# scverse/squidpy

Measured on AMD Instinct MI355X. Metric: nhood_enrichment permutations/sec (1e6 spots x 30 clusters), higher is better.
Workload: dtype u8 labels / u32 counts / i64 moments; 1 GPU; nhood_enrichment: 1000000 spots (1000x1000 hex grid, nnz=5992002), 30 clusters, 10000 permutations per step per GPU, on-device Philox-keyed label shuffles; collective=none

## Files before the change

### squidpy_amd/csrc/sqgr_nhood.hip

```cpp
#include "sqgr_common.h"
#include "sqgr_rng.h"
#include "sqgr_shuffle.h"
#include "sqgr_pcg.h"

#include <algorithm>
#include <cstdlib>
#include <type_traits>

namespace sqgr {

constexpr int COUNT_THREADS = 1024;
constexpr size_t LDS_BUDGET = 160 * 1024;

__host__ __device__ constexpr int key_words_per_row(int B, int n_libs) {
    return n_libs * ((B / FEISTEL_GROUP) * 8 + (B / 2) * 2) < (B / 2) * 8 ? (B / 2) * 8 : n_libs * ((B / FEISTEL_GROUP) * 8 + (B / 2) * 2);
}

__global__ void k_keygen(uint64_t seed, int64_t perm0, int nrows, int B, int n_libs, uint32_t* __restrict__ keys) {
    const int items = B / FEISTEL_GROUP + B / 2;
    const int64_t t = blockIdx.x * (int64_t)blockDim.x + threadIdx.x;
    if (t >= (int64_t)nrows * n_libs * items) return;
    const int item = (int)(t % items);
    const uint32_t lib = (uint32_t)((t / items) % n_libs);
    const int64_t row = t / ((int64_t)items * n_libs);
// ... 55 lines not shown
    if (pw == 16) {
        *reinterpret_cast<uint4*>(batch_base + (size_t)i * 16) = make_uint4(w0, w1, w2, w3);
    } else if (pw == 8) {
        *reinterpret_cast<uint2*>(batch_base + (size_t)i * 8) = make_uint2(w0, w1);
        *reinterpret_cast<uint2*>(batch_base + (size_t)n * 8 + (size_t)i * 8) = make_uint2(w2, w3);
    } else if (pw == 4) {
        uint32_t* d = reinterpret_cast<uint32_t*>(batch_base) + i;
        d[0] = w0; d[(size_t)n] = w1; d[(size_t)2 * n] = w2; d[(size_t)3 * n] = w3;
    } else if (pw == 2) {
        uint16_t* d = reinterpret_cast<uint16_t*>(batch_base) + i;
        const uint32_t w[4] = {w0, w1, w2, w3};
#pragma unroll
        for (int q = 0; q < 8; ++q) d[(size_t)q * n] = (uint16_t)(w[q >> 1] >> (16 * (q & 1)));
    } else {
        uint8_t* d = batch_base + i;
        const uint32_t w[4] = {w0, w1, w2, w3};
#pragma unroll
        for (int q = 0; q < 16; ++q) d[(size_t)q * n] = (uint8_t)(w[q >> 2] >> (8 * (q & 3)));
    }
}

template <int B, bool HAS_LIBS, bool SMALLK>
__global__ __launch_bounds__(256) void k_shuffle(int64_t n, const uint32_t* __restrict__ cum, int kpad, int blk_words, int K,
                                                 const uint32_t* __restrict__ keys, LibDom dom0, int n_libs, int nrows,
                                                 const int32_t* __restrict__ lib_of, const int32_t* __restrict__ rank_of,
                                                 const LibDom* __restrict__ libdoms, uint8_t* __restrict__ slab_all, int pw,
                                                 const int32_t* __restrict__ spot_of) {
    extern __shared__ uint32_t s_lds[];
    uint32_t* s_cum = s_lds + blk_words;
    for (int t = threadIdx.x; t < n_libs * kpad; t += 256) s_cum[t] = cum[t];
    for (int t = threadIdx.x; t < blk_words; t += 256) s_lds[t] = cum[n_libs * kpad + t];
    __syncthreads();
    constexpr int NG = B / FEISTEL_GROUP;
    const int row0 = (NG == 2) ? blockIdx.y : 2 * blockIdx.y;
    const int row1 = (NG == 2) ? row0 : min(row0 + 1, nrows - 1);
    const bool store1 = (NG == 2) || row0 + 1 < nrows;
    const size_t row_words = key_words_per_row(B, n_libs);
    const uint32_t* kgA = keys + (size_t)row0 * row_words;
    const uint32_t* kgB = (NG == 2) ? kgA + (size_t)n_libs * 8 : keys + (size_t)row1 * row_words;
    const uint32_t* ksA = keys + (size_t)row0 * row_words + (size_t)NG * n_libs * 8;
    const uint32_t* ksB = (NG == 2) ? ksA + (size_t)(FEISTEL_GROUP / 2) * n_libs * 2
                                    : keys + (size_t)row1 * row_words + (size_t)NG * n_libs * 8;
    const uint32_t zero = 0;
    const uint32_t sent_add = (uint32_t)(128 - K) * 0x01010101u;
    for (int64_t i = blockIdx.x * (int64_t)blockDim.x + threadIdx.x; i < n; i += (int64_t)gridDim.x * blockDim.x) {
    LibDom ld = dom0;
    uint32_t x0 = (uint32_t)i, lib = 0;
    if (HAS_LIBS) {
        lib = (uint32_t)lib_of[i];
        ld = libdoms[lib];
        x0 = (uint32_t)rank_of[i];
    } else if (spot_of) {
        x0 = (uint32_t)spot_of[i];
    }
    const FeistelDomain dom = ld.dom;
    const uint32_t* tab = s_cum + lib * kpad + 1;
    typedef __attribute__((address_space(3))) const uint32_t lds_word;
    const uint32_t blk_base = HAS_LIBS ? ld.aoff * 4u : 0u;
    auto blk_at = [&](uint32_t byte_off) { return *reinterpret_cast<lds_word*>((uintptr_t)(blk_base + byte_off)); };
    const uint32_t a0 = x0 / dom.B, b0 = x0 - a0 * dom.B;

    u16x2 ga = (u16x2)((unsigned short)a0), gb = (u16x2)((unsigned short)b0);
    {
        uint32_t kp[8];
#pragma unroll
        for (int r = 0; r < 8; ++r) kp[r] = (kgA[(size_t)lib * 8 + r] & 0xFFFFu) | (kgB[(size_t)lib * 8 + r] & 0xFFFF0000u);
        const uint32_t* const pg[1] = {kp};
        bool need0 = true, need1 = true;
        do {
            u16x2 na[1] = {ga}, nb[1] = {gb};
            feistel_rounds<1>(na, nb, dom, pg);
            if (need0) { ga.x = na[0].x; gb.x = nb[0].x; }
            if (need1) { ga.y = na[0].y; gb.y = nb[0].y; }
            need0 = __umul24((uint32_t)ga.x, dom.B) + (uint32_t)gb.x >= dom.n;
            need1 = __umul24((uint32_t)ga.y, dom.B) + (uint32_t)gb.y >= dom.n;
        } while (need0 | need1);
    }
    auto emit_group = [&](const u16x2 gsa, const u16x2 gsb, const uint32_t* ks, uint32_t (&out)[4]) {
#pragma unroll
        for (int w = 0; w < FEISTEL_GROUP / 4; ++w) {
            uint32_t word = 0;
            uint32_t apk[2], bpk[2];
#pragma unroll
            for (int jj = 0; jj < 2; ++jj) {
                const uint32_t* const pk[1] = {ks + ((size_t)(w * 2 + jj) * n_libs + lib) * 2};
                u16x2 a[1] = {gsa}, b[1] = {gsb};
                sigma_rounds<1>(a, b, dom, pk);
                apk[jj] = __builtin_bit_cast(uint32_t, a[0]);
                bpk[jj] = __builtin_bit_cast(uint32_t, b[0]);
                const uint32_t a4 = apk[jj] << 2;
                const uint32_t e0 = blk_at(a4 & 0xFFFFu);
                const uint32_t e1 = blk_at(a4 >> 16);
                if (jj == 0) {
                    put_label<0, 0>(word, e0, bpk[jj], zero);
                    put_label<1, 1>(word, e1, bpk[jj], zero);
                } else {
                    put_label<2, 0>(word, e0, bpk[jj], zero);
                    put_label<3, 1>(word, e1, bpk[jj], zero);
                }
            }
            bool sentinel;
            if constexpr (SMALLK) {
                sentinel = ((word + sent_add) & 0x80808080u) != 0;
            } else {
                const uint32_t k = (uint32_t)K;
                sentinel = k > 255u || (word & 0xFFu) >= k || ((word >> 8) & 0xFFu) >= k || ((word >> 16) & 0xFFu) >= k || (word >> 24) >= k;
            }
            if (sentinel) {
#pragma unroll
                for (int j = 0; j < 4; ++j) {
                    if (K <= 255 && ((word >> (8 * j)) & 0xFFu) < (uint32_t)K) continue;
                    const int jj = j >> 1, sh = (j & 1) * 16;
                    const uint32_t* sk = ks + ((size_t)(w * 2 + jj) * n_libs + lib) * 2;
                    const uint32_t k0 = (sk[0] >> sh) & 0xFFFFu, k1 = (sk[1] >> sh) & 0xFFFFu;
                    uint32_t a = (apk[jj] >> sh) & 0xFFFFu, b = (bpk[jj] >> sh) & 0xFFFFu;
                    uint32_t x = a * dom.B + b;
                    while (x >= dom.n) {
                        uint32_t t = b + feistel_F1(a, k0, dom.bsh);
                        t = t >= dom.B ? t - dom.B : t;
                        b = t >= dom.B ? t - dom.B : t;
                        a = (a + feistel_F1(b, k1, dom.ash)) & (dom.A - 1u);
                        x = a * dom.B + b;
                    }
                    const uint32_t e = blk_at(a * 4u);
                    uint32_t l = (e & 0xFFFFu) + (b >= (e >> 16) ? 1u : 0u);
                    if (l >= (uint32_t)K) {
                        l = K <= 255 ? (e >> 8) & 0xFFu : 0u;
                        while (x >= tab[l]) ++l;
                    }
                    word = (word & ~(0xFFu << (8 * j))) | (l << (8 * j));
                }
            }
            out[w] = word;
        }
    };
    uint32_t outA[4], outB[4];
    emit_group((u16x2)(ga.x), (u16x2)(gb.x), ksA, outA);
    if (store1) emit_group((u16x2)(ga.y), (u16x2)(gb.y), ksB, outB);
    if constexpr (NG == 2) {
        uint4* dst = reinterpret_cast<uint4*>(slab_all + ((size_t)row0 * n + i) * B);
        dst[0] = make_uint4(outA[0], outA[1], outA[2], outA[3]);
        dst[1] = make_uint4(outB[0], outB[1], outB[2], outB[3]);
    } else {
        slab_store16(slab_all + (size_t)row0 * n * 16, n, i, pw, outA[0], outA[1], outA[2], outA[3]);
        if (store1) slab_store16(slab_all + (size_t)row1 * n * 16, n, i, pw, outB[0], outB[1], outB[2], outB[3]);
    }
    }
}

constexpr int SHUF_TAB_THREADS = 1024;
constexpr uint32_t SHUF_TAB_MAX_A = 1024;
constexpr int SHUF_TAB_BLOCKS_PER_CU = 20;
constexpr int SHUF_TAB_MIN_TRIPS = 16;
template <bool SMALLK>
__global__ __launch_bounds__(SHUF_TAB_THREADS, 8) void k_shuffle_tab(int64_t n, const uint32_t* __restrict__ cum, int kpad, int blk_words, int K,
                                                                  const uint32_t* __restrict__ keys, LibDom dom0, int nrows,
                                                                  uint8_t* __restrict__ slab_all, int pw, const int32_t* __restrict__ spot_of,
                                                                  int tab_word0) {
    extern __shared__ uint32_t s_lds[];
    uint32_t* s_cum = s_lds + blk_words;
    for (int t = threadIdx.x; t < kpad; t += SHUF_TAB_THREADS) s_cum[t] = cum[t];
    for (int t = threadIdx.x; t < blk_words; t += SHUF_TAB_THREADS) s_lds[t] = cum[kpad + t];
    const FeistelDomain dom = dom0.dom;
    const int row0 = 2 * blockIdx.y;
    const int row1 = min(row0 + 1, nrows - 1);
    const bool store1 = row0 + 1 < nrows;
    constexpr size_t row_words = key_words_per_row(16, 1);
    const uint32_t* kgA = keys + (size_t)row0 * row_words;
    const uint32_t* kgB = keys + (size_t)row1 * row_words;
    const uint32_t* ksA = kgA + 8;
    const uint32_t* ksB = kgB + 8;
    const u16x2 BB = (u16x2)((unsigned short)dom.B);
    {
        const u16x2 bsh = (u16x2)((unsigned short)dom.bsh);
        const int words = (int)dom.A * 8;
        for (int idx = threadIdx.x; idx < words; idx += SHUF_TAB_THREADS) {
            const u16x2 av = (u16x2)((unsigned short)(idx >> 3));
            const int t = idx & 7;
            u16x2 fa = feistel_F2(av, __builtin_bit_cast(u16x2, ksA[t * 2]), bsh);
            u16x2 fb = feistel_F2(av, __builtin_bit_cast(u16x2, ksB[t * 2]), bsh);
            fa = __builtin_elementwise_min(fa, (u16x2)(fa - BB));
            fb = __builtin_elementwise_min(fb, (u16x2)(fb - BB));
            s_lds[tab_word0 + idx] = __builtin_bit_cast(uint32_t, fa);
            s_lds[tab_word0 + words + idx] = __builtin_bit_cast(uint32_t, fb);
        }
    }
    __syncthreads();
    const uint32_t zero = 0;
    const uint32_t sent_add = (uint32_t)(128 - K) * 0x01010101u;
    const uint32_t* tab = s_cum + 1;
    typedef __attribute__((address_space(3))) const uint32_t lds_word;
    typedef uint32_t u32x4 __attribute__((ext_vector_type(4)));
    typedef __attribute__((address_space(3))) const u32x4 lds_row;
    auto blk_at = [&](uint32_t byte_off) { return *reinterpret_cast<lds_word*>((uintptr_t)byte_off); };
    const uint32_t tabA = (uint32_t)tab_word0 * 4u, tabB = tabA + dom.A * 32u;
    const u16x2 am = (u16x2)((unsigned short)(dom.A - 1u));
    const u16x2 ash = (u16x2)((unsigned short)dom.ash);
    for (int64_t i = blockIdx.x * (int64_t)SHUF_TAB_THREADS + threadIdx.x; i < n; i += (int64_t)gridDim.x * SHUF_TAB_THREADS) {
    const uint32_t x0 = spot_of ? (uint32_t)spot_of[i] : (uint32_t)i;
    const uint32_t a0 = x0 / dom.B, b0 = x0 - a0 * dom.B;
    u16x2 ga = (u16x2)((unsigned short)a0), gb = (u16x2)((unsigned short)b0);
    {
        uint32_t kp[8];
#pragma unroll
        for (int r = 0; r < 8; ++r) kp[r] = (kgA[r] & 0xFFFFu) | (kgB[r] & 0xFFFF0000u);
        const uint32_t* const pg[1] = {kp};
        bool need0 = true, need1 = true;
        do {
            u16x2 na[1] = {ga}, nb[1] = {gb};
            feistel_rounds<1>(na, nb, dom, pg);
            if (need0) { ga.x = na[0].x; gb.x = nb[0].x; }
            if (need1) { ga.y = na[0].y; gb.y = nb[0].y; }
            need0 = __umul24((uint32_t)ga.x, dom.B) + (uint32_t)gb.x >= dom.n;
            need1 = __umul24((uint32_t)ga.y, dom.B) + (uint32_t)gb.y >= dom.n;
        } while (need0 | need1);
    }
    auto emit_group = [&](const u16x2 gsa, const u16x2 gsb, const uint32_t row_off, const uint32_t* ks, uint32_t (&out)[4]) {
        const u32x4 r0 = *reinterpret_cast<lds_row*>((uintptr_t)row_off);
        const u32x4 r1 = *reinterpret_cast<lds_row*>((uintptr_t)(row_off + 16u));
        const uint32_t f1[8] = {r0.x, r0.y, r0.z, r0.w, r1.x, r1.y, r1.z, r1.w};
#pragma unroll
        for (int w = 0; w < FEISTEL_GROUP / 4; ++w) {
            uint32_t word = 0;
            uint32_t apk[2], bpk[2];
#pragma unroll
            for (int jj = 0; jj < 2; ++jj) {
                const u16x2 t = gsb + __builtin_bit_cast(u16x2, f1[w * 2 + jj]);
                const u16x2 b = __builtin_elementwise_min(t, (u16x2)(t - BB));
                const u16x2 k1 = __builtin_bit_cast(u16x2, ks[(w * 2 + jj) * 2 + 1]);
                const u16x2 a = (gsa + feistel_F2(b, k1, ash)) & am;
                apk[jj] = __builtin_bit_cast(uint32_t, a);
                bpk[jj] = __builtin_bit_cast(uint32_t, b);
                const uint32_t a4 = apk[jj] << 2;
                const uint32_t e0 = blk_at(a4 & 0xFFFFu);
                const uint32_t e1 = blk_at(a4 >> 16);
                if (jj == 0) {
                    put_label<0, 0>(word, e0, bpk[jj], zero);
                    put_label<1, 1>(word, e1, bpk[jj], zero);
                } else {
                    put_label<2, 0>(word, e0, bpk[jj], zero);
                    put_label<3, 1>(word, e1, bpk[jj], zero);
                }
            }
            bool sentinel;
            if constexpr (SMALLK) {
                sentinel = ((word + sent_add) & 0x80808080u) != 0;
            } else {
                const uint32_t k = (uint32_t)K;
                sentinel = k > 255u || (word & 0xFFu) >= k || ((word >> 8) & 0xFFu) >= k || ((word >> 16) & 0xFFu) >= k || (word >> 24) >= k;
            }
            if (sentinel) {
#pragma unroll
                for (int j = 0; j < 4; ++j) {
                    if (K <= 255 && ((word >> (8 * j)) & 0xFFu) < (uint32_t)K) continue;
                    const int jj = j >> 1, sh = (j & 1) * 16;
                    const uint32_t* sk = ks + (w * 2 + jj) * 2;
                    uint32_t a = (apk[jj] >> sh) & 0xFFFFu, b = (bpk[jj] >> sh) & 0xFFFFu;
                    uint32_t x = a * dom.B + b;
                    if (x >= dom.n) {
                        const uint32_t k0 = (sk[0] >> sh) & 0xFFFFu, k1 = (sk[1] >> sh) & 0xFFFFu;
                        do {
                            uint32_t t = b + feistel_F1(a, k0, dom.bsh);
                            t = t >= dom.B ? t - dom.B : t;
                            b = t >= dom.B ? t - dom.B : t;
                            a = (a + feistel_F1(b, k1, dom.ash)) & (dom.A - 1u);
                            x = a * dom.B + b;
                        } while (x >= dom.n);
                    }
                    const uint32_t e = blk_at(a * 4u);
                    uint32_t l = (e & 0xFFFFu) + (b >= (e >> 16) ? 1u : 0u);
                    if (l >= (uint32_t)K) {
                        l = K <= 255 ? (e >> 8) & 0xFFu : 0u;
                        while (x >= tab[l]) ++l;
                    }
                    word = (word & ~(0xFFu << (8 * j))) | (l << (8 * j));
                }
            }
            out[w] = word;
        }
    };
    uint32_t outA[4], outB[4];
    emit_group((u16x2)(ga.x), (u16x2)(gb.x), tabA + (uint32_t)ga.x * 32u, ksA, outA);
    if (store1) emit_group((u16x2)(ga.y), (u16x2)(gb.y), tabB + (uint32_t)ga.y * 32u, ksB, outB);
    slab_store16(slab_all + (size_t)row0 * n * 16, n, i, pw, outA[0], outA[1], outA[2], outA[3]);
    if (store1) slab_store16(slab_all + (size_t)row1 * n * 16, n, i, pw, outB[0], outB[1], outB[2], outB[3]);
    }
}

template <bool SMALLK>
__global__ __launch_bounds__(256) void k_shuffle_indep(int64_t n, const uint32_t* __restrict__ cum, int kpad, int blk_words, int K,
                                                       const uint32_t* __restrict__ keys, LibDom dom0, uint8_t* __restrict__ slab_all, int pw) {
    extern __shared__ uint32_t s_lds[];
    uint32_t* s_cum = s_lds + blk_words;
    for (int t = threadIdx.x; t < kpad; t += 256) s_cum[t] = cum[t];
    for (int t = threadIdx.x; t < blk_words; t += 256) s_lds[t] = cum[kpad + t];
    __syncthreads();
    const int row = blockIdx.y;
    const uint32_t* krow = keys + (size_t)row * key_words_per_row(16, 1);
    const uint32_t zero = 0;
    const uint32_t sent_add = (uint32_t)(128 - K) * 0x01010101u;
    const FeistelDomain dom = dom0.dom;
    const uint32_t* tab = s_cum + 1;
    typedef __attribute__((address_space(3))) const uint32_t lds_word;
    auto blk_at = [&](uint32_t byte_off) { return *reinterpret_cast<lds_word*>((uintptr_t)byte_off); };
    for (int64_t i = blockIdx.x * (int64_t)blockDim.x + threadIdx.x; i < n; i += (int64_t)gridDim.x * blockDim.x) {
        const uint32_t x0 = (uint32_t)i;
        const uint32_t a0 = x0 / dom.B, b0 = x0 - a0 * dom.B;
        uint32_t out[4];
#pragma unroll
        for (int w = 0; w < 4; ++w) {
            uint32_t word = 0, apk[2], bpk[2];
#pragma unroll
            for (int jj = 0; jj < 2; ++jj) {
                const uint32_t* const pk[1] = {krow + (w * 2 + jj) * 8};
                u16x2 ga = (u16x2)((unsigned short)a0), gb = (u16x2)((unsigned short)b0);
                bool need0 = true, need1 = true;
                do {
                    u16x2 na[1] = {ga}, nb[1] = {gb};
                    feistel_rounds<1>(na, nb, dom, pk);
                    if (need0) { ga.x = na[0].x; gb.x = nb[0].x; }
                    if (need1) { ga.y = na[0].y; gb.y = nb[0].y; }
                    need0 = __umul24((uint32_t)ga.x, dom.B) + (uint32_t)gb.x >= dom.n;
                    need1 = __umul24((uint32_t)ga.y, dom.B) + (uint32_t)gb.y >= dom.n;
                } while (need0 | need1);
                apk[jj] = __builtin_bit_cast(uint32_t, ga);
                bpk[jj] = __builtin_bit_cast(uint32_t, gb);
                const uint32_t a4 = apk[jj] << 2;
                const uint32_t e0 = blk_at(a4 & 0xFFFFu);
                const uint32_t e1 = blk_at(a4 >> 16);
                if (jj == 0) {
                    put_label<0, 0>(word, e0, bpk[jj], zero);
                    put_label<1, 1>(word, e1, bpk[jj], zero);
                } else {
                    put_label<2, 0>(word, e0, bpk[jj], zero);
                    put_label<3, 1>(word, e1, bpk[jj], zero);
                }
            }
            bool sentinel;
            if constexpr (SMALLK) {
                sentinel = ((word + sent_add) & 0x80808080u) != 0;
            } else {
                const uint32_t k = (uint32_t)K;
                sentinel = k > 255u || (word & 0xFFu) >= k || ((word >> 8) & 0xFFu) >= k || ((word >> 16) & 0xFFu) >= k || (word >> 24) >= k;
            }
            if (sentinel) {
#pragma unroll
                for (int j = 0; j < 4; ++j) {
                    if (K <= 255 && ((word >> (8 * j)) & 0xFFu) < (uint32_t)K) continue;
                    const int jj = j >> 1, sh = (j & 1) * 16;
                    const uint32_t a = (apk[jj] >> sh) & 0xFFFFu, b = (bpk[jj] >> sh) & 0xFFFFu;
                    const uint32_t x = a * dom.B + b;
                    const uint32_t e = blk_at(a * 4u);
                    uint32_t l = (e & 0xFFFFu) + (b >= (e >> 16) ? 1u : 0u);
                    if (l >= (uint32_t)K) {
                        l = K <= 255 ? (e >> 8) & 0xFFu : 0u;
                        while (x >= tab[l]) ++l;
                    }
                    word = (word & ~(0xFFu << (8 * j))) | (l << (8 * j));
                }
            }
            out[w] = word;
        }
        slab_store16(slab_all + (size_t)row * n * 16, n, i, pw, out[0], out[1], out[2], out[3]);
    }
}

template <bool HAS_LIBS>
__global__ __launch_bounds__(256) void k_shuffle16(int64_t n, const uint32_t* __restrict__ cum, int kpad, int blk_words, int K,
                                                   const uint32_t* __restrict__ keys, LibDom dom0, int n_libs,
                                                   const int32_t* __restrict__ lib_of, const int32_t* __restrict__ rank_of,
                                                   const LibDom* __restrict__ libdoms, uint16_t* __restrict__ slab_all, int tab_lds) {
    extern __shared__ uint32_t s_lds[];
    uint32_t* s_cum = s_lds + blk_words;
    if (tab_lds)
        for (int t = threadIdx.x; t < n_libs * kpad; t += 256) s_cum[t] = cum[t];
    for (int t = threadIdx.x; t < blk_words; t += 256) s_lds[t] = cum[n_libs * kpad + t];
    __syncthreads();
    constexpr int B = 16;
    const int batch = blockIdx.y;
    const uint32_t* kg = keys + (size_t)batch * key_words_per_row(B, n_libs);
    const uint32_t* ks = kg + (size_t)n_libs * 8;
    for (int64_t i = blockIdx.x * (int64_t)blockDim.x + threadIdx.x; i < n; i += (int64_t)gridDim.x * blockDim.x) {
        LibDom ld = dom0;
        uint32_t x0 = (uint32_t)i, lib = 0;
        if (HAS_LIBS) {
            lib = (uint32_t)lib_of[i];
            ld = libdoms[lib];
            x0 = (uint32_t)rank_of[i];
        }
        const FeistelDomain dom = ld.dom;
        const uint32_t* tab = s_cum + lib * kpad + 1;
        const uint32_t* gtab = cum + lib * kpad + 1;
        const uint32_t* blk = s_lds + ld.aoff;
        uint32_t ga = x0 / dom.B, gb = x0 - ga * dom.B;
        const uint32_t* gk = kg + (size_t)lib * 8;
        do {
            for (int r = 0; r < FEISTEL_ROUNDS; r += 2) {
                ga = (ga + feistel_F1(gb, gk[r], dom.ash)) & (dom.A - 1u);
                uint32_t t = gb + feistel_F1(ga, gk[r + 1], dom.bsh);
                t = t >= dom.B ? t - dom.B : t;
                gb = t >= dom.B ? t - dom.B : t;
            }
        } while (ga * dom.B + gb >= dom.n);
        uint32_t out[B / 2];
#pragma unroll
        for (int j = 0; j < B; ++j) {
            const uint32_t* sk = ks + ((size_t)(j >> 1) * n_libs + lib) * 2;
            const int sh = (j & 1) * 16;
            const uint32_t k0 = (sk[0] >> sh) & 0xFFFFu, k1 = (sk[1] >> sh) & 0xFFFFu;
            uint32_t a = ga, b = gb, x;
            do {
                uint32_t t = b + feistel_F1(a, k0, dom.bsh);
                t = t >= dom.B ? t - dom.B : t;
                b = t >= dom.B ? t - dom.B : t;
                a = (a + feistel_F1(b, k1, dom.ash)) & (dom.A - 1u);
                x = a * dom.B + b;
            } while (x >= dom.n);
            const uint32_t e = blk[a];
            uint32_t l = (e & 0xFFFFu) + (b >= (e >> 16) ? 1u : 0u);
            if (l >= (uint32_t)K) {
                uint32_t lo = 0, hi = (uint32_t)K - 1u;
                if (tab_lds) {
                    while (lo < hi) {
                        const uint32_t mid = (lo + hi) >> 1;
                        if (x < tab[mid]) hi = mid; else lo = mid + 1;
                    }
                } else {
                    while (lo < hi) {
                        const uint32_t mid = (lo + hi) >> 1;
                        if (x < gtab[mid]) hi = mid; else lo = mid + 1;
                    }
                }
                l = lo;
            }
            if (j & 1) out[j >> 1] |= l << 16; else out[j >> 1] = l;
        }
// ... 1652 lines not shown
                        if (events == 0) { ev_label = (uint32_t)K; ev_pos = n_l - lo; }
                        ++events;
                    }
                    if (events == 0)
                        word = lab | (0xFFFFu << 16);
                    else if (events == 1 && ev_label == lab + 1 && ev_pos > 0)
                        word = lab | ((uint32_t)ev_pos << 16);
                    else
                        word = SENT | (K <= 255 ? lab << 8 : 0u);
                }
                blk[doms[l].aoff + a] = word;
            }
        }
        const size_t cum_words = cum.size();
        cum.insert(cum.end(), blk.begin(), blk.end());
        (void)cum_words;
        if (!libs_on) p->dom0 = doms[0];
        {
            std::vector<uint32_t> off((size_t)p->n_libs + 1, 0);
            for (int l = 0; l < p->n_libs; ++l) off[l + 1] = off[l] + (uint32_t)cnt[l];
            std::vector<uint8_t> base((size_t)n, 0);
            if (labels)
                for (int64_t i = 0; i < n; ++i) base[libs_on ? off[lib_ids[i]] + (uint32_t)rank[i] : (uint32_t)i] = (uint8_t)labels[i];
            p->has_labels = labels != nullptr;
            if (K > 256 && labels) {
                std::vector<uint16_t> b16((size_t)n, 0);
                for (int64_t i = 0; i < n; ++i) b16[libs_on ? off[lib_ids[i]] + (uint32_t)rank[i] : (uint32_t)i] = (uint16_t)labels[i];
                if ((rc = p->base16.alloc((size_t)n)) != SQGR_OK) break;
                if (hipMemcpy(p->base16.p, b16.data(), (size_t)n * 2, hipMemcpyHostToDevice) != hipSuccess) { rc = SQGR_ERR_HIP; break; }
            }
            if ((rc = p->base_pos.alloc((size_t)n)) != SQGR_OK) break;
            if ((rc = p->lib_off.alloc(off.size())) != SQGR_OK) break;
            hipError_t e2 = hipMemcpy(p->base_pos.p, base.data(), (size_t)n, hipMemcpyHostToDevice);
            if (e2 == hipSuccess) e2 = hipMemcpy(p->lib_off.p, off.data(), off.size() * 4, hipMemcpyHostToDevice);
            if (e2 != hipSuccess) {
                set_error("label upload failed: %s", hipGetErrorString(e2));
                rc = SQGR_ERR_HIP;
                break;
            }
        }
        if ((rc = p->cum.alloc(cum.size())) != SQGR_OK) break;
        hipError_t e = hipMemcpy(p->cum.p, cum.data(), cum.size() * 4, hipMemcpyHostToDevice);
        if (e == hipSuccess && libs_on) {
            if ((rc = p->lib_of.alloc((size_t)n)) != SQGR_OK) break;
            if ((rc = p->rank_of.alloc((size_t)n)) != SQGR_OK) break;
            if ((rc = p->libs.alloc((size_t)n_libs)) != SQGR_OK) break;
            e = hipMemcpy(p->lib_of.p, lib_ids, (size_t)n * 4, hipMemcpyHostToDevice);
            if (e == hipSuccess) e = hipMemcpy(p->rank_of.p, rank.data(), (size_t)n * 4, hipMemcpyHostToDevice);
            if (e == hipSuccess) e = hipMemcpy(p->libs.p, doms.data(), (size_t)n_libs * sizeof(LibDom), hipMemcpyHostToDevice);
        }
        if (e != hipSuccess) {
            set_error("label upload failed: %s", hipGetErrorString(e));
            rc = SQGR_ERR_HIP;
        }
    } while (0);
    if (rc != SQGR_OK) {
        delete p;
        return rc;
    }
    *out_plan = p;
    return SQGR_OK;
}

int sqgr_nhood_create(sqgr_ctx* ctx, const sqgr_graph* g, const int32_t* labels, int32_t K, const int32_t* lib_ids,
                      int32_t n_libs, sqgr_nhood** out_plan) {
    SQGR_REQUIRE(ctx && g && out_plan, "ctx/graph/out_plan is NULL");
    return nhood_build(ctx, g, g->n, labels, K, lib_ids, n_libs, out_plan);
}

int sqgr_nhood_destroy(sqgr_nhood* plan) {
    if (!plan) return SQGR_OK;
    (void)hipSetDevice(plan->ctx->device);
    delete plan;
    return SQGR_OK;
}

int sqgr_nhood_tune(sqgr_nhood* plan, int32_t perms_per_pass, int32_t blocks_per_batch, int32_t batches_per_launch) {
    SQGR_REQUIRE(plan, "plan is NULL");
    SQGR_REQUIRE(perms_per_pass == 0 || perms_per_pass == 16 || perms_per_pass == 32 || perms_per_pass == 8 || perms_per_pass == 4 ||
                     perms_per_pass == 2 || perms_per_pass == 1,
                 "perms_per_pass must be 0, 32, 16 (slab width) or 8, 4, 2, 1 (cap of the LDS pass width of a 16-wide slab)");
    SQGR_REQUIRE(blocks_per_batch >= 0 && blocks_per_batch <= 65535 && batches_per_launch >= 0 && batches_per_launch <= 1024,
                 "tuning value out of range");
    plan->B = perms_per_pass == 32 ? 32 : 16;
    plan->pass_cap = (perms_per_pass > 0 && perms_per_pass < 16) ? perms_per_pass : 16;
    plan->nblk = blocks_per_batch;
    plan->nbatch = batches_per_launch;
    plan->keys.release(); plan->slab.release(); plan->partial.release(); plan->acc_sum.release(); plan->acc_sq.release();
    return SQGR_OK;
}

static int launch_shuffle_raw(sqgr_nhood* p, int B, int nb, const uint32_t* keys, uint8_t* slab, hipStream_t st, int pw = 16) {
    unsigned gx = (unsigned)ceil_div(p->n, 256);
    int per_cu = 96;
    const char* env_blocks = getenv("SQGR_SHUFFLE_BLOCKS_PER_CU");
    if (env_blocks && atoi(env_blocks) > 0) per_cu = atoi(env_blocks);
    gx = std::min<unsigned>(gx, (unsigned)(per_cu * std::max(p->ctx->cu_count, 1)) / (unsigned)std::max(nb, 1) + 1);
    LaunchTimer t(p->ctx, p->wide() ? "nhood_shuffle16" : "nhood_shuffle", st);
    const size_t lds = (p->tab_lds ? (size_t)p->n_libs * p->kpad * 4 : 0) + (size_t)p->blk_bytes * 4;
    if (p->wide()) {
        if (B != 16) {
            set_error("more than 256 clusters: 16 permutations per pass only");
            return SQGR_ERR_UNSUPPORTED;
        }
        uint16_t* slab16 = reinterpret_cast<uint16_t*>(slab);
        if (p->has_libs) {
            SQGR_TRY(allow_lds(k_shuffle16<true>, lds));
            k_shuffle16<true><<<dim3(gx, nb), 256, lds, st>>>(p->n, p->cum.p, p->kpad, p->blk_bytes, p->K, keys, p->dom0, p->n_libs, p->lib_of.p,
                                                              p->rank_of.p, p->libs.p, slab16, p->tab_lds ? 1 : 0);
        } else {
            SQGR_TRY(allow_lds(k_shuffle16<false>, lds));
            k_shuffle16<false><<<dim3(gx, nb), 256, lds, st>>>(p->n, p->cum.p, p->kpad, p->blk_bytes, p->K, keys, p->dom0, p->n_libs, p->lib_of.p,
                                                               p->rank_of.p, p->libs.p, slab16, p->tab_lds ? 1 : 0);
        }
        SQGR_HIP(hipGetLastError());
        return SQGR_OK;
    }
    if (p->independent) {
        if (B != 16 || p->has_libs) {
            set_error("SQGR_SHUFFLE_INDEPENDENT: 16 permutations per row and no libraries only");
            return SQGR_ERR_UNSUPPORTED;
        }
        if (p->K <= 126) k_shuffle_indep<true><<<dim3(gx, nb), 256, lds, st>>>(p->n, p->cum.p, p->kpad, p->blk_bytes, p->K, keys, p->dom0, slab, pw);
        else k_shuffle_indep<false><<<dim3(gx, nb), 256, lds, st>>>(p->n, p->cum.p, p->kpad, p->blk_bytes, p->K, keys, p->dom0, slab, pw);
        SQGR_HIP(hipGetLastError());
        return SQGR_OK;
    }
    const unsigned gy = (unsigned)(B == 32 ? nb : (nb + 1) / 2);
    {
        const char* env_tab = getenv("SQGR_SHUFFLE_TABLE");
        const int mode = env_tab ? atoi(env_tab) : -1;
        const uint32_t A = p->dom0.dom.A;
        const size_t tab_word0 = (lds / 4 + 7) & ~(size_t)7;
        const size_t lds_tab = tab_word0 * 4 + (size_t)2 * A * 32;
        const char* why = nullptr;
        if (B != 16) why = "32 permutations per row";
        else if (p->has_libs) why = "libraries (per-library domains and keys)";
        else if (A > SHUF_TAB_MAX_A) why = "more than 2^20 spots (high digit A > 1024: the two tables exceed 64 KB)";
        else if (lds_tab > LDS_BUDGET / 2) why = "tables do not fit two blocks per CU";
        if (mode == 2 && why) {
            set_error("SQGR_SHUFFLE_TABLE=2: the table kernel does not take this input: %s", why);
            return SQGR_ERR_UNSUPPORTED;
        }
        const int cus = std::max(p->ctx->cu_count, 1);
        const int64_t block_trips = ceil_div(p->n, SHUF_TAB_THREADS) * (int64_t)gy;
        const bool big = block_trips >= (int64_t)SHUF_TAB_MIN_TRIPS * 2 * cus;
        if (!why && mode != 0 && (mode == 1 || mode == 2 || big)) {
            int tab_per_cu = SHUF_TAB_BLOCKS_PER_CU;
            if (env_blocks && atoi(env_blocks) > 0) tab_per_cu = atoi(env_blocks);
            const unsigned nblk = (unsigned)ceil_div(p->n, SHUF_TAB_THREADS);
            const unsigned cap = (unsigned)(tab_per_cu * cus) / gy + 1;
            const unsigned trips = (nblk + cap - 1) / cap;
            const unsigned tx = (nblk + trips - 1) / trips;
            if (p->K <= 126) {
                SQGR_TRY(allow_lds(k_shuffle_tab<true>, lds_tab));
                k_shuffle_tab<true><<<dim3(tx, gy), SHUF_TAB_THREADS, lds_tab, st>>>(p->n, p->cum.p, p->kpad, p->blk_bytes, p->K, keys, p->dom0, nb, slab, pw,
                                                                                   p->spot_of.p, (int)tab_word0);
            } else {
                SQGR_TRY(allow_lds(k_shuffle_tab<false>, lds_tab));
                k_shuffle_tab<false><<<dim3(tx, gy), SHUF_TAB_THREADS, lds_tab, st>>>(p->n, p->cum.p, p->kpad, p->blk_bytes, p->K, keys, p->dom0, nb, slab, pw,
                                                                                    p->spot_of.p, (int)tab_word0);
            }
            SQGR_HIP(hipGetLastError());
            return SQGR_OK;
        }
    }
#define SQGR_SHUFFLE(BB, LIBS, SK)                                                                                             \
    k_shuffle<BB, LIBS, SK><<<dim3(gx, gy), 256, lds, st>>>(p->n, p->cum.p, p->kpad, p->blk_bytes, p->K, keys, p->dom0, p->n_libs, nb, \
                                                            p->lib_of.p, p->rank_of.p, p->libs.p, slab, pw, p->spot_of.p)
#define SQGR_SHUFFLE_K(BB, LIBS) \
    if (p->K <= 126) SQGR_SHUFFLE(BB, LIBS, true); else SQGR_SHUFFLE(BB, LIBS, false)
    if (B == 32) {
        if (p->has_libs) { SQGR_SHUFFLE_K(32, true); } else { SQGR_SHUFFLE_K(32, false); }
    } else {
        if (p->has_libs) { SQGR_SHUFFLE_K(16, true); } else { SQGR_SHUFFLE_K(16, false); }
    }
#undef SQGR_SHUFFLE_K
#undef SQGR_SHUFFLE
    SQGR_HIP(hipGetLastError());
    return SQGR_OK;
}

static int launch_shuffle(sqgr_nhood* p, int nb, int buf, hipStream_t st) {
    return launch_shuffle_raw(p, p->B, nb, p->keys.p + (size_t)buf * p->keys_stride(), p->slab.p + (size_t)buf * p->slab_stride(), st, p->plane_w());
}

int sqgr_nhood_run(sqgr_nhood* plan, uint64_t seed, int64_t perm_begin, int64_t perm_end, const int64_t* shift,
                   int64_t* out_sum, uint64_t* out_sumsq, uint32_t* out_perms) {
    SQGR_REQUIRE(plan && out_sum && out_sumsq, "plan/out_sum/out_sumsq is NULL");
    SQGR_REQUIRE(perm_begin >= 0 && perm_end >= perm_begin, "bad permutation range [%lld,%lld)", (long long)perm_begin,
                 (long long)perm_end);
    sqgr_nhood* p = plan;
    sqgr_ctx* ctx = p->ctx;
    SQGR_HIP(hipSetDevice(ctx->device));
    hipStream_t st = ctx->stream;
    const int K2 = p->K2;
    const int64_t nperm = perm_end - perm_begin;
    {
        const char* e = getenv("SQGR_SHUFFLE_INDEPENDENT");
        p->independent = e && atoi(e) == 1;
        SQGR_REQUIRE(!p->independent || (p->B == 16 && !p->has_libs && !p->wide()), "SQGR_SHUFFLE_INDEPENDENT needs 16-wide rows, K <= 256 and no libraries");
        SQGR_REQUIRE(!p->independent || !p->mapped(), "SQGR_SHUFFLE_INDEPENDENT: no spot map");
    }
    auto local = [&]() -> int {
    SQGR_TRY(p->ensure_workspace(out_perms != nullptr));
    const int B = p->B, hw = p->acc_words();
    const int64_t per_launch = (int64_t)p->nbatch * B;
    if (shift)
        SQGR_HIP(hipMemcpyAsync(p->shift.p, shift, (size_t)K2 * 8, hipMemcpyHostToDevice, st));
    else
        SQGR_HIP(hipMemsetAsync(p->shift.p, 0, (size_t)K2 * 8, st));
    SQGR_HIP(hipMemsetAsync(p->acc_sum.p, 0, (size_t)p->nbatch * hw * 8, st));
    SQGR_HIP(hipMemsetAsync(p->acc_sq.p, 0, (size_t)p->nbatch * hw * 8, st));
    if (out_perms && nperm > 0) SQGR_TRY(p->perms_dev.ensure((size_t)nperm * K2));
    const char* env_streams = getenv("SQGR_NHOOD_STREAMS");
    hipStream_t sa = (env_streams && atoi(env_streams) == 2) ? ctx->stream2 : st;
    int64_t grp = 0;
    for (int64_t p0 = perm_begin - perm_begin % FEISTEL_GROUP; p0 < perm_end; p0 += per_launch, ++grp) {
        const int64_t todo = (perm_end - p0 < per_launch) ? perm_end - p0 : per_launch;
        const int nb = (int)ceil_div(todo, B);
        const int buf = (sa != st) ? (int)(grp & 1) : 0;
        if (sa != st && grp >= 2) SQGR_HIP(hipStreamWaitEvent(sa, p->ev_counted[buf], 0));
        {
            LaunchTimer t(ctx, "nhood_keygen", sa);
            const int64_t nk = (int64_t)nb * p->n_libs * (B / FEISTEL_GROUP + B / 2);
            if (p->independent)
                k_keygen_indep<<<(unsigned)ceil_div((int64_t)nb * 8, 256), 256, 0, sa>>>(seed, p0, nb, p->keys.p + (size_t)buf * p->keys_stride());
            else
                k_keygen<<<(unsigned)ceil_div(nk, 256), 256, 0, sa>>>(seed, p0, nb, B, p->n_libs, p->keys.p + (size_t)buf * p->keys_stride());
            SQGR_HIP(hipGetLastError());
        }
        SQGR_TRY(launch_shuffle(p, nb, buf, sa));
        SQGR_HIP(hipEventRecord(p->ev_shuffled[buf], sa));
        SQGR_HIP(hipStreamWaitEvent(st, p->ev_shuffled[buf], 0));
        p->columns_valid = p->has_labels;
        const int rc_count = p->count_batches(nb, buf);
        p->columns_valid = false;
        SQGR_TRY(rc_count);
        SQGR_TRY(p->reduce_batches(nb, p0, perm_begin, perm_end, out_perms ? p->perms_dev.p : nullptr));
        SQGR_HIP(hipEventRecord(p->ev_counted[buf], st));
    }
    {
        LaunchTimer t(ctx, "nhood_finalize");
        SQGR_HIP(hipMemsetAsync(p->fin.p, 0, (size_t)2 * K2 * 8, st));
        k_finalize<<<(unsigned)ceil_div(hw, 256), 256, 0, st>>>(p->acc_sum.p, p->acc_sq.p, p->nbatch, hw, p->acc_pw(), K2, p->fin.p,
                                                               reinterpret_cast<uint64_t*>(p->fin.p + K2));
        SQGR_HIP(hipGetLastError());
    }
    return SQGR_OK;
    };
    SQGR_TRY(comm_agree(p->comm, local(), st));
    SQGR_TRY(comm_allreduce_i64_dev(p->comm, p->fin.p, (size_t)2 * K2, false, st));
    SQGR_HIP(hipMemcpyAsync(out_sum, p->fin.p, (size_t)K2 * 8, hipMemcpyDeviceToHost, st));
    SQGR_HIP(hipMemcpyAsync(out_sumsq, p->fin.p + K2, (size_t)K2 * 8, hipMemcpyDeviceToHost, st));
    if (out_perms && nperm > 0)
        SQGR_HIP(hipMemcpyAsync(out_perms, p->perms_dev.p, (size_t)nperm * K2 * 4, hipMemcpyDeviceToHost, st));
    SQGR_HIP(hipStreamSynchronize(st));
    return SQGR_OK;
}

int sqgr_nhood_shuffled_labels(sqgr_nhood* plan, uint64_t seed, int64_t perm, uint8_t* out_labels) {
    SQGR_REQUIRE(plan && out_labels && perm >= 0, "plan/out_labels is NULL or perm < 0");
    SQGR_REQUIRE(plan->K <= 256, "sqgr_nhood_shuffled_labels returns uint8 labels: K=%d > 256", plan->K);
    SQGR_REQUIRE(!plan->mapped(), "a plan with a spot map (sqgr_nhood_set_spot_map) runs sqgr_nhood_run only");
    sqgr_nhood* p = plan;
    sqgr_ctx* ctx = p->ctx;
    SQGR_HIP(hipSetDevice(ctx->device));
    SQGR_TRY(p->ensure_workspace(false));
    hipStream_t st = ctx->stream;
    const int B = p->B;
    const int64_t perm_row = perm - perm % FEISTEL_GROUP;
    {
        const char* e = getenv("SQGR_SHUFFLE_INDEPENDENT");
        p->independent = e && atoi(e) == 1;
        SQGR_REQUIRE(!p->independent || (B == 16 && !p->has_libs && !p->wide()), "SQGR_SHUFFLE_INDEPENDENT needs 16-wide rows, K <= 256 and no libraries");
    }
    if (p->independent)
        k_keygen_indep<<<1, 256, 0, st>>>(seed, perm_row, 1, p->keys.p);
    else
        k_keygen<<<(unsigned)ceil_div((int64_t)p->n_libs * (B / FEISTEL_GROUP + B / 2), 256), 256, 0, st>>>(seed, perm_row, 1, B, p->n_libs,
                                                                                                           p->keys.p);
    SQGR_HIP(hipGetLastError());
    SQGR_TRY(launch_shuffle(p, 1, 0, st));
    std::vector<uint8_t> rows((size_t)p->n * B);
    SQGR_HIP(hipMemcpyAsync(rows.data(), p->slab.p, rows.size(), hipMemcpyDeviceToHost, st));
    SQGR_HIP(hipStreamSynchronize(st));
    const int pw = p->plane_w(), slot = (int)(perm - perm_row);
    for (int64_t i = 0; i < p->n; ++i)
        out_labels[i] = pw == 16 || B != 16 ? rows[(size_t)i * B + (size_t)slot]
                                            : rows[(size_t)(slot / pw) * p->n * pw + (size_t)i * pw + (size_t)(slot % pw)];
    return SQGR_OK;
}

int sqgr_nhood_counts_batch(sqgr_ctx* ctx, const sqgr_graph* g, const uint8_t* labels, int64_t n_perms, int32_t K,
                            uint32_t* out_counts) {
    SQGR_REQUIRE(ctx && g && labels && out_counts, "ctx/graph/labels/out is NULL");
    SQGR_REQUIRE(n_perms >= 0, "n_perms < 0");
    SQGR_REQUIRE(K <= 256, "sqgr_nhood_counts_batch takes uint8 labels: K=%d > 256", K);
    const int64_t n = g->n;
    for (int64_t t = 0; t < n_perms * n; ++t)
        SQGR_REQUIRE(labels[t] < K, "labels[%lld]=%d outside [0,%d)", (long long)t, (int)labels[t], K);
    sqgr_nhood* p = nullptr;
    SQGR_TRY(sqgr_nhood_create(ctx, g, nullptr, K, nullptr, 0, &p));
    int rc = SQGR_OK;
    do {
        if ((rc = p->ensure_workspace(true)) != SQGR_OK) break;
        const int B = p->B, K2 = p->K2, hw = p->acc_words();
        const int64_t per_launch = (int64_t)p->nbatch * B;
        hipStream_t st = ctx->stream;
        if ((rc = p->stage.ensure((size_t)per_launch * n)) != SQGR_OK) break;
        if ((rc = p->perms_dev.ensure((size_t)(n_perms > 0 ? n_perms : 1) * K2)) != SQGR_OK) break;
        hipError_t e = hipMemsetAsync(p->shift.p, 0, (size_t)K2 * 8, st);
        if (e == hipSuccess) e = hipMemsetAsync(p->acc_sum.p, 0, (size_t)p->nbatch * hw * 8, st);
        if (e == hipSuccess) e = hipMemsetAsync(p->acc_sq.p, 0, (size_t)p->nbatch * hw * 8, st);
        for (int64_t p0 = 0; p0 < n_perms && e == hipSuccess && rc == SQGR_OK; p0 += per_launch) {
// ... 318 lines not shown
```

Baseline: 1.209 million permutations/s.

## Streamline table shuffle kernel: hoisted keys, strength-reduced index split, pre-scaled digit

Specialises the table-based shuffle kernel on whether a spot map is present. Without a map it replaces the per-iteration division of the spot index by an incremental digit update. Round keys are packed once per thread outside the grid-stride loop, and the Feistel rounds use a custom unrolled helper with a register-pinned multiplier constant. The first loop trip runs unconditionally, leaving the cycle-walk as an unlikely branch. The high digit is carried pre-scaled by 4 so LDS lookups skip a shift, and the first label byte is written by inline SDWA assembly. This also narrows the loop index to 32 bits and ties correctness to the static assert on table size.

```diff
diff --git a/squidpy_amd/csrc/sqgr_nhood.hip b/squidpy_amd/csrc/sqgr_nhood.hip
--- a/squidpy_amd/csrc/sqgr_nhood.hip
+++ b/squidpy_amd/csrc/sqgr_nhood.hip
@@ -231,7 +231,36 @@
 constexpr uint32_t SHUF_TAB_MAX_A = 1024;
 constexpr int SHUF_TAB_BLOCKS_PER_CU = 20;
 constexpr int SHUF_TAB_MIN_TRIPS = 16;
-template <bool SMALLK>
+static_assert(SHUF_TAB_MAX_A * 4u <= (1u << 12), "k_shuffle_tab carries the high digit scaled by 4 in a 16-bit half: ash - 2 >= 4, a << 2 < 2^12");
+
+__device__ __forceinline__ u16x2 shuf_tab_F2(u16x2 v, u16x2 k, u16x2 sh, u16x2 c1) {
+    u16x2 x = v * c1 + k;
+    x ^= x >> (u16x2)(7);
+    x *= (u16x2)(FEISTEL_C2);
+    return x >> sh;
+}
+__device__ __forceinline__ void shuf_tab_rounds(u16x2& a, u16x2& b, const uint32_t (&kp)[8], u16x2 am, u16x2 ash, u16x2 bsh, u16x2 BB,
+                                                u16x2 c1) {
+#pragma unroll
+    for (int r = 0; r < FEISTEL_ROUNDS; r += 2) {
+        a = (a + shuf_tab_F2(b, __builtin_bit_cast(u16x2, kp[r]), ash, c1)) & am;
+        u16x2 t = b + shuf_tab_F2(a, __builtin_bit_cast(u16x2, kp[r + 1]), bsh, c1);
+        t = __builtin_elementwise_min(t, (u16x2)(t - BB));
+        b = __builtin_elementwise_min(t, (u16x2)(t - BB));
+    }
+}
+__device__ __forceinline__ uint32_t first_label(uint32_t e, uint32_t bpk, uint32_t zero) {
+    uint32_t word;
+    asm("v_cmp_le_u32_sdwa vcc, %1, %2 src0_sel:WORD_1 src1_sel:WORD_0\n\t"
+        "v_addc_co_u32_sdwa %0, vcc, %1, %3, vcc dst_sel:BYTE_0 dst_unused:UNUSED_PAD src0_sel:BYTE_0 src1_sel:DWORD\n\t"
+        "s_nop 0"
+        : "=v"(word)
+        : "v"(e), "v"(bpk), "v"(zero)
+        : "vcc");
+    return word;
+}
+
+template <bool SMALLK, bool NOMAP>
 __global__ __launch_bounds__(SHUF_TAB_THREADS, 8) void k_shuffle_tab(int64_t n, const uint32_t* __restrict__ cum, int kpad, int blk_words, int K,
                                                                   const uint32_t* __restrict__ keys, LibDom dom0, int nrows,
                                                                   uint8_t* __restrict__ slab_all, int pw, const int32_t* __restrict__ spot_of,
@@ -274,47 +303,73 @@
     auto blk_at = [&](uint32_t byte_off) { return *reinterpret_cast<lds_word*>((uintptr_t)byte_off); };
     const uint32_t tabA = (uint32_t)tab_word0 * 4u, tabB = tabA + dom.A * 32u;
     const u16x2 am = (u16x2)((unsigned short)(dom.A - 1u));
-    const u16x2 ash = (u16x2)((unsigned short)dom.ash);
-    for (int64_t i = blockIdx.x * (int64_t)SHUF_TAB_THREADS + threadIdx.x; i < n; i += (int64_t)gridDim.x * SHUF_TAB_THREADS) {
-    const uint32_t x0 = spot_of ? (uint32_t)spot_of[i] : (uint32_t)i;
-    const uint32_t a0 = x0 / dom.B, b0 = x0 - a0 * dom.B;
+    const u16x2 ash = (u16x2)((unsigned short)dom.ash), bsh = (u16x2)((unsigned short)dom.bsh);
+    const u16x2 am4 = (u16x2)((unsigned short)((dom.A - 1u) << 2));
+    const u16x2 ash4 = (u16x2)((unsigned short)(dom.ash - 2u));
+    uint32_t c1w = FEISTEL_C1 * 0x10001u;
+    asm volatile("" : "+v"(c1w));
+    const u16x2 c1 = __builtin_bit_cast(u16x2, c1w);
+    const uint32_t n32 = (uint32_t)n, stride = gridDim.x * (uint32_t)SHUF_TAB_THREADS;
+    uint32_t i = blockIdx.x * (uint32_t)SHUF_TAB_THREADS + threadIdx.x;
+    uint32_t sa = 0, sb = 0, a0 = 0, b0 = 0;
+    if constexpr (NOMAP) {
+        sa = stride / dom.B;
+        sb = stride - sa * dom.B;
+        asm volatile("" : "+v"(sa), "+v"(sb));
+        a0 = i / dom.B;
+        b0 = i - a0 * dom.B;
+    }
+    uint32_t kp[8];
+#pragma unroll
+    for (int r = 0; r < 8; ++r) {
+        kp[r] = (kgA[r] & 0xFFFFu) | (kgB[r] & 0xFFFF0000u);
+        asm volatile("" : "+v"(kp[r]));
+    }
+    for (; i < n32; i += stride) {
+    if constexpr (!NOMAP) {
+        const uint32_t x0 = (uint32_t)spot_of[i];
+        a0 = x0 / dom.B;
+        b0 = x0 - a0 * dom.B;
+    }
     u16x2 ga = (u16x2)((unsigned short)a0), gb = (u16x2)((unsigned short)b0);
     {
-        uint32_t kp[8];
-#pragma unroll
-        for (int r = 0; r < 8; ++r) kp[r] = (kgA[r] & 0xFFFFu) | (kgB[r] & 0xFFFF0000u);
-        const uint32_t* const pg[1] = {kp};
-        bool need0 = true, need1 = true;
-        do {
-            u16x2 na[1] = {ga}, nb[1] = {gb};
-            feistel_rounds<1>(na, nb, dom, pg);
-            if (need0) { ga.x = na[0].x; gb.x = nb[0].x; }
-            if (need1) { ga.y = na[0].y; gb.y = nb[0].y; }
+        shuf_tab_rounds(ga, gb, kp, am, ash, bsh, BB, c1);
+        bool need0 = __umul24((uint32_t)ga.x, dom.B) + (uint32_t)gb.x >= dom.n;
+        bool need1 = __umul24((uint32_t)ga.y, dom.B) + (uint32_t)gb.y >= dom.n;
+        while (__builtin_expect(need0 | need1, 0)) {
+            u16x2 na = ga, nb = gb;
+            shuf_tab_rounds(na, nb, kp, am, ash, bsh, BB, c1);
+            if (need0) { ga.x = na.x; gb.x = nb.x; }
+            if (need1) { ga.y = na.y; gb.y = nb.y; }
             need0 = __umul24((uint32_t)ga.x, dom.B) + (uint32_t)gb.x >= dom.n;
             need1 = __umul24((uint32_t)ga.y, dom.B) + (uint32_t)gb.y >= dom.n;
-        } while (need0 | need1);
-    }
-    auto emit_group = [&](const u16x2 gsa, const u16x2 gsb, const uint32_t row_off, const uint32_t* ks, uint32_t (&out)[4]) {
+        }
+    }
+    if constexpr (NOMAP) {
+        a0 += sa;
+        b0 += sb;
+        if (b0 >= dom.B) { b0 -= dom.B; ++a0; }
+    }
+    auto emit_group = [&](const uint32_t ga1, const uint32_t gb1, const uint32_t row_off, const uint32_t* ks, uint32_t (&out)[4]) {
+        const u16x2 gsa4 = (u16x2)((unsigned short)(ga1 << 2)), gsb = (u16x2)((unsigned short)gb1);
         const u32x4 r0 = *reinterpret_cast<lds_row*>((uintptr_t)row_off);
         const u32x4 r1 = *reinterpret_cast<lds_row*>((uintptr_t)(row_off + 16u));
         const uint32_t f1[8] = {r0.x, r0.y, r0.z, r0.w, r1.x, r1.y, r1.z, r1.w};
 #pragma unroll
         for (int w = 0; w < FEISTEL_GROUP / 4; ++w) {
-            uint32_t word = 0;
-            uint32_t apk[2], bpk[2];
+            uint32_t word;
+            uint32_t a4pk[2], bpk[2];
 #pragma unroll
             for (int jj = 0; jj < 2; ++jj) {
                 const u16x2 t = gsb + __builtin_bit_cast(u16x2, f1[w * 2 + jj]);
                 const u16x2 b = __builtin_elementwise_min(t, (u16x2)(t - BB));
                 const u16x2 k1 = __builtin_bit_cast(u16x2, ks[(w * 2 + jj) * 2 + 1]);
-                const u16x2 a = (gsa + feistel_F2(b, k1, ash)) & am;
-                apk[jj] = __builtin_bit_cast(uint32_t, a);
                 bpk[jj] = __builtin_bit_cast(uint32_t, b);
-                const uint32_t a4 = apk[jj] << 2;
-                const uint32_t e0 = blk_at(a4 & 0xFFFFu);
-                const uint32_t e1 = blk_at(a4 >> 16);
+                a4pk[jj] = __builtin_bit_cast(uint32_t, (u16x2)((gsa4 + shuf_tab_F2(b, k1, ash4, c1)) & am4));
+                const uint32_t e0 = blk_at(a4pk[jj] & 0xFFFFu);
+                const uint32_t e1 = blk_at(a4pk[jj] >> 16);
                 if (jj == 0) {
-                    put_label<0, 0>(word, e0, bpk[jj], zero);
+                    word = first_label(e0, bpk[jj], zero);
                     put_label<1, 1>(word, e1, bpk[jj], zero);
                 } else {
                     put_label<2, 0>(word, e0, bpk[jj], zero);
@@ -334,7 +389,7 @@
                     if (K <= 255 && ((word >> (8 * j)) & 0xFFu) < (uint32_t)K) continue;
                     const int jj = j >> 1, sh = (j & 1) * 16;
                     const uint32_t* sk = ks + (w * 2 + jj) * 2;
-                    uint32_t a = (apk[jj] >> sh) & 0xFFFFu, b = (bpk[jj] >> sh) & 0xFFFFu;
+                    uint32_t a = ((a4pk[jj] >> sh) & 0xFFFFu) >> 2, b = (bpk[jj] >> sh) & 0xFFFFu;
                     uint32_t x = a * dom.B + b;
                     if (x >= dom.n) {
                         const uint32_t k0 = (sk[0] >> sh) & 0xFFFFu, k1 = (sk[1] >> sh) & 0xFFFFu;
@@ -359,8 +414,8 @@
         }
     };
     uint32_t outA[4], outB[4];
-    emit_group((u16x2)(ga.x), (u16x2)(gb.x), tabA + (uint32_t)ga.x * 32u, ksA, outA);
-    if (store1) emit_group((u16x2)(ga.y), (u16x2)(gb.y), tabB + (uint32_t)ga.y * 32u, ksB, outB);
+    emit_group((uint32_t)ga.x, (uint32_t)gb.x, tabA + (uint32_t)ga.x * 32u, ksA, outA);
+    if (store1) emit_group((uint32_t)ga.y, (uint32_t)gb.y, tabB + (uint32_t)ga.y * 32u, ksB, outB);
     slab_store16(slab_all + (size_t)row0 * n * 16, n, i, pw, outA[0], outA[1], outA[2], outA[3]);
     if (store1) slab_store16(slab_all + (size_t)row1 * n * 16, n, i, pw, outB[0], outB[1], outB[2], outB[3]);
     }
@@ -2319,15 +2374,18 @@
             const unsigned cap = (unsigned)(tab_per_cu * cus) / gy + 1;
             const unsigned trips = (nblk + cap - 1) / cap;
             const unsigned tx = (nblk + trips - 1) / trips;
+#define SQGR_SHUFFLE_TAB(SK, NOMAP)                                                                                             \
+    do {                                                                                                                       \
+        SQGR_TRY(allow_lds(k_shuffle_tab<SK, NOMAP>, lds_tab));                                                                \
+        k_shuffle_tab<SK, NOMAP><<<dim3(tx, gy), SHUF_TAB_THREADS, lds_tab, st>>>(p->n, p->cum.p, p->kpad, p->blk_bytes, p->K, keys, p->dom0, nb, \
+                                                                                slab, pw, p->spot_of.p, (int)tab_word0);        \
+    } while (0)
             if (p->K <= 126) {
-                SQGR_TRY(allow_lds(k_shuffle_tab<true>, lds_tab));
-                k_shuffle_tab<true><<<dim3(tx, gy), SHUF_TAB_THREADS, lds_tab, st>>>(p->n, p->cum.p, p->kpad, p->blk_bytes, p->K, keys, p->dom0, nb, slab, pw,
-                                                                                   p->spot_of.p, (int)tab_word0);
+                if (p->spot_of.p) SQGR_SHUFFLE_TAB(true, false); else SQGR_SHUFFLE_TAB(true, true);
             } else {
-                SQGR_TRY(allow_lds(k_shuffle_tab<false>, lds_tab));
-                k_shuffle_tab<false><<<dim3(tx, gy), SHUF_TAB_THREADS, lds_tab, st>>>(p->n, p->cum.p, p->kpad, p->blk_bytes, p->K, keys, p->dom0, nb, slab, pw,
-                                                                                    p->spot_of.p, (int)tab_word0);
-            }
+                if (p->spot_of.p) SQGR_SHUFFLE_TAB(false, false); else SQGR_SHUFFLE_TAB(false, true);
+            }
+#undef SQGR_SHUFFLE_TAB
             SQGR_HIP(hipGetLastError());
             return SQGR_OK;
         }
```

Measured after the change: 1.262 million permutations/s, median of 6. +4.4%, better.
